# wangyunpeng139/3_ORB_SLAM3_SelfNote

Measured on AMD Instinct MI355X. Metric: frames/sec ORB extract+match, 752x480, higher is better.
Workload: dtype u8; 1 GPU; BASELINE configs[2]: extract + SearchByProjection match, 1000x1000 candidates, synthetic frame stream; image=752x480, nfeatures=1000, nlevels=8, batch=256, distinct_frames_per_gpu=2048, streams=4

## Files before the change

3_orb_slam3_selfnote_amd/csrc/orb_common.h:

```cpp
#pragma once
#include <stdint.h>
#include <stddef.h>

#define ORB_EDGE_THRESHOLD 19
#define ORB_PATCH_SIZE 31
#define ORB_HALF_PATCH 15
#define ORB_MIN_BORDER 16
#define ORB_DISC_PIXELS 749
#define ORB_MAXL 16

#define FAST_TILE_PITCH 80
#define FAST_TILE_COLS 65
#define FAST_TILE_ROWS 76
#define FAST_S_PITCH 64

#define FAST_REC_WORDS 32
#define FAST_REC_GROUP_WORDS 8
#define FAST_REC_CELL_WORDS 4

#define RESIZE_ROWS_MAX 16
#define RESIZE_REC_GROUP_WORDS 4
#define RESIZE_REC_WORDS (RESIZE_REC_GROUP_WORDS + 4 * RESIZE_ROWS_MAX)

#define BLUR_TILE_INTERIOR 0x100u
#define BLUR_TILE_WHOLE_STORES 0x200u

#ifndef ORB_DESCRIBE_K
#define ORB_DESCRIBE_K 8
#endif
#define ORB_DESCRIBE_GROUPS(totalKp, K) ((((totalKp) + (K) - 1) / (K) + 3) / 4 > 1 ? (((totalKp) + (K) - 1) / (K) + 3) / 4 : 1)

__host__ __device__ constexpr int clamp_count(int n, int cap) { return (n > 0 ? n : 0) < cap ? (n > 0 ? n : 0) : cap; }
static_assert(clamp_count(-1, 8) == 0 && clamp_count(0, 8) == 0 && clamp_count(5, 8) == 5 && clamp_count(8, 8) == 8 && clamp_count(9, 8) == 8, "clamp_count");
static_assert(clamp_count(-1, 0) == 0 && clamp_count(0, 0) == 0 && clamp_count(1, 0) == 0, "clamp_count: cap == 0");

struct LiveCount {
  const int32_t *dev; int stride; int konst;
  __device__ __forceinline__ int at(int p, int cap) const { return dev ? clamp_count(dev[(size_t)p * stride], cap) : konst; }
};

struct LevelGeom {
  int w, h;
  int pitch;
  int bpitch;
  size_t off;
  size_t boff;
  int maxBorderX, maxBorderY;
  int nCols, nRows, wCell, hCell;
  int cellCap;
  int cellBase;
  int slotBase;
  int N;
  int nIni;
  float hX;
  int candBase;
  int candCap;
  int kpBase, kpCap;
  float scale;
  float kpsize;
  int xtabBase, ytabBase;
  int resizeRows;
  int resizeSrcRows;
  int resizeTPitch;
  int resizeRecBase;
  int tilesX, tilesY, tileBase;
  uint32_t rowTileMagic;
};

#define CHAIN_TILE 32
#define CHAIN_NT 1024
struct ChainTile {
  uint16_t level, pad;
  uint16_t x[ORB_MAXL], y[ORB_MAXL], w[ORB_MAXL], h[ORB_MAXL];
};

struct FrameParams {
  LevelGeom geom[ORB_MAXL];
  int nlevels;
  int nframes;
  int iniTh, minTh;
  int lap0, lap1;
  const uint8_t *img0;
  size_t img0_stride, img0_frame_stride;
  uint8_t *pyr;    size_t pyr_fs;
  uint8_t *blur;   size_t blur_fs;
  uint32_t *cellCnt; int cell_fs;
  uint32_t *slots;   size_t slot_fs;
  uint32_t *cand;    int cand_fs;
  uint16_t *knode;
  uint32_t *lkp;     int lkp_fs;
  uint16_t *lrank;
  int32_t *lcnt;
  int32_t *candCnt;
  const int2 *xtab, *ytab;
  const int8_t *disc;
  const uint32_t *tiles;
  uint32_t magicCells, magicTiles, magicKpBlk;
  int totalTiles;
  int totalCells;
  int totalGroups;
  uint32_t magicGroups;
  const uint32_t *fastRecs;
  const uint32_t *resizeRecs;
  int totalKp;
  int octCap;
  const ChainTile *chain;
  int chainBuf0, chainBuf1;
  void *out_kps;
  uint8_t *out_desc;
  int32_t *out_counts;
  int cap;
};
```

3_orb_slam3_selfnote_amd/csrc/orb_kernels.h:

```cpp
#pragma once
#include <hip/hip_runtime.h>
#include <type_traits>
#include "orb_common.h"
#include "orb_fast_score.h"
#include "orb_sincos.h"

#define WAVE 64

__constant__ __attribute__((aligned(16))) int8_t c_pattern[1024] = {
#include "../../include/orb_pattern_data.inc"
};

struct DiscTab { uint32_t w[64][6]; };
constexpr int kDiscUmax[16] = {15, 15, 15, 15, 14, 14, 14, 13, 13, 12, 11, 10, 9, 8, 6, 3};
constexpr DiscTab make_disc_tab() {
  DiscTab t{};
  int n = 0;
  for (int v = -15; v <= 15; v++) {
    const int d = kDiscUmax[v < 0 ? -v : v];
    for (int u = -d; u <= d; u++) {
      const int lane = n & 63, k = n >> 6;
      t.w[lane][k >> 2] |= (uint32_t)(uint8_t)(int8_t)u << (8 * (k & 3));
      t.w[lane][3 + (k >> 2)] |= (uint32_t)(uint8_t)(int8_t)v << (8 * (k & 3));
      n++;
// ... 530 lines not shown
        const unsigned long long bK = __builtin_amdgcn_ballot_w64(keep);
        const uint32_t rank = (uint32_t)nkept + (uint32_t)lane_rank(bK);
        if (keep && rank < cellCap) slots[rank] = ((uint32_t)(S - 1) << 24) | yxv;
        nkept += __popcll(bK);
      };
      for (int y0 = 0; y0 < ch; y0 += 2 * rpi, off += 2 * stepB, yr += 2 * rpi, yx += (uint32_t)rpi << 13) {
        const int SA = sS[off], SB = sS[off + stepB];
        const bool candA = ((tt - SA) & yr) < 0, candB = ((tt - SB) & (yr + rpi)) < 0;
        const unsigned long long bA = __builtin_amdgcn_ballot_w64(candA), bB = __builtin_amdgcn_ballot_w64(candB);
        if (bA != 0ull) walk(candA, SA, off, y0 + sub, yx);
        if (bB != 0ull) walk(candB, SB, off + stepB, y0 + rpi + sub, yx + ((uint32_t)rpi << 12));
      }
    }
    FSTAMP(2);
    if (nkept > 0 || detection == 1 || P.minTh >= P.iniTh) break;
    t = P.minTh;
    wave_lds_order();
  }
  if (lane == 0) *cellCnt = (uint32_t)min(nkept, (int)cellCap);
  FSTAMP(7);
}

#ifdef OCT_STAMPS
#define OSTAMP(i) do { const long long t_ = __builtin_readcyclecounter(); if (threadIdx.x == 0 && g_fast_stamps) g_fast_stamps[(size_t)blockIdx.x * 8 + (i)] += (unsigned int)(t_ - ot0); ot0 = t_; } while (0)
#else
#define OSTAMP(i) do {} while (0)
#endif
struct OctNode { short ulx, urx, uly, bry; };

#ifndef OCT_REGKEYS
#define OCT_REGKEYS 4096
#endif
template <int NT, bool CELLS_LDS>
__global__ __launch_bounds__(NT) void k_octree(FrameParams P, uint32_t *cellOffScratch) {
  extern __shared__ __align__(16) uint8_t smem[];
#ifdef OCT_STAMPS
  long long ot0 = __builtin_readcyclecounter();
#endif
  const int CAP = P.octCap;
  unsigned long long *best = reinterpret_cast<unsigned long long *>(smem);
  uint32_t *chcnt = reinterpret_cast<uint32_t *>(smem);
  int32_t *chpos = reinterpret_cast<int32_t *>(smem + 16 * (size_t)CAP);
  OctNode *nodeA = reinterpret_cast<OctNode *>(smem + 32 * (size_t)CAP);
  OctNode *nodeB = nodeA + CAP;
  uint32_t *cntA = reinterpret_cast<uint32_t *>(nodeB + CAP);
  uint32_t *cntB = cntA + CAP;
  int32_t *npos = reinterpret_cast<int32_t *>(cntB + CAP);
  int32_t *rankOf = npos + CAP;
  uint32_t *incl = reinterpret_cast<uint32_t *>(rankOf + CAP);
  uint32_t *sflag = incl + CAP;
  uint32_t *sw = sflag + CAP;
  __shared__ int shI[8];

  const int tid = threadIdx.x, lane = tid & 63, wid = tid >> 6;
  constexpr int NW = NT / 64;
  const int level = (int)(blockIdx.x / (unsigned)P.nframes), frame = (int)(blockIdx.x - (unsigned)level * (unsigned)P.nframes);
  const LevelGeom G = P.geom[level];
  int32_t *lcnt = P.lcnt + ((size_t)frame * P.nlevels + level) * 2;
  uint32_t *cand = P.cand + (size_t)frame * P.cand_fs + G.candBase;
  uint16_t *knode = P.knode + (size_t)frame * P.cand_fs + G.candBase;
  constexpr int PER = OCT_REGKEYS / NT, REGN = PER * NT;
  uint32_t rc[PER > 0 ? PER : 1], rk[PER > 0 ? PER : 1];
#pragma unroll
  for (int j = 0; j < PER; j++) { rc[j] = 0u; rk[j] = 0u; }
  auto for_keys = [&](int n_, auto f) {
#pragma unroll
    for (int j = 0; j < PER; j++) {
      if (j * NT >= n_) break;
      const int k = tid + j * NT;
      if (k < n_) f(k, rc[j], rk[j]);
    }
    for (int k = REGN + tid; k < n_; k += NT) {
      uint32_t c = cand[k], nd = knode[k];
      f(k, c, nd);
      knode[k] = (uint16_t)nd;
    }
  };

  const int ncell = G.nCols * G.nRows;
  const uint32_t *cellCnt = P.cellCnt + (size_t)frame * P.cell_fs + G.cellBase;
  uint32_t *cellOffG = cellOffScratch + (size_t)frame * P.cell_fs + G.cellBase;
  uint32_t *cellOffL = sw + (NT / 64 + 2);
  uint32_t carry = 0;
  for (int base = 0; base < ncell; base += NT) {
    int i = base + tid;
// ... 25 lines not shown
          const int mid = (lo + hi + 1) >> 1;
          if (cellOffL[mid] <= (uint32_t)k) lo = mid; else hi = mid - 1;
        }
        return slots[(size_t)lo * G.cellCap + ((uint32_t)k - cellOffL[lo])];
      };
#pragma unroll
      for (int j = 0; j < PER; j++) {
        if (j * NT >= n) break;
        const int k = tid + j * NT;
        if (k < n) { rc[j] = fetch(k); cand[k] = rc[j]; }
      }
      for (int k = REGN + tid; k < n; k += NT) cand[k] = fetch(k);
      __syncthreads();
    } else {
      for (int cidx = wid; cidx < ncell; cidx += NW) {
        uint32_t cnt = cellCnt[cidx], off = cellOffG[cidx];
        for (uint32_t j = lane; j < cnt; j += 64)
          if (off + j < (uint32_t)n) cand[off + j] = slots[(size_t)cidx * G.cellCap + j];
      }
      __syncthreads();
#pragma unroll
      for (int j = 0; j < PER; j++) {
        if (j * NT >= n) break;
        const int k = tid + j * NT;
        if (k < n) rc[j] = cand[k];
      }
    }
  }
  OSTAMP(0);

  const int nIni = G.nIni;
  const float hX = G.hX;
  const int Hrect = G.maxBorderY - ORB_MIN_BORDER;
  for (int i = tid; i < nIni; i += NT) chcnt[i] = 0;
  __syncthreads();
  for_keys(n, [&](int, uint32_t &c, uint32_t &nd) {
    int r = (int)((float)(c & 0xfff) / hX);
    r = min(max(r, 0), nIni - 1);
    nd = (uint32_t)r;
    atomicAdd(&chcnt[r], 1u);
  });
  __syncthreads();
  if (tid == 0) {
    int L = 0;
    for (int r = 0; r < nIni; r++) {
      uint32_t cn = chcnt[r];
      if (cn > 0) {
        OctNode nd;
        nd.ulx = (short)(int)(hX * (float)r);
        nd.urx = (short)(int)(hX * (float)(r + 1));
        nd.uly = 0;
        nd.bry = (short)Hrect;
        nodeA[L] = nd;
        cntA[L] = cn;
        chpos[r] = L;
        L++;
      }
    }
    shI[0] = L;
  }
  __syncthreads();
  for_keys(n, [&](int, uint32_t &, uint32_t &nd) { nd = (uint32_t)chpos[nd]; });
  int L = shI[0];
  __syncthreads();
  OSTAMP(1);

  const int N = G.N;
  bool careful = false;
  OctNode *nodes = nodeA, *nodesN = nodeB;
  uint32_t *cnts = cntA, *cntsN = cntB;
  for (int guard = 0; guard < 64; guard++) {
    const int prevSize = L;
    for (int i = tid; i < 4 * L; i += NT) chcnt[i] = 0;
    if (tid == 0) { shI[1] = 0; shI[2] = 0x7fffffff; }
    __syncthreads();
    for_keys(n, [&](int, uint32_t &c, uint32_t &nd) {
      if (cnts[nd] > 1) {
        OctNode o = nodes[nd];
        int x = c & 0xfff, y = (c >> 12) & 0xfff;
        int hx = (o.urx - o.ulx + 1) >> 1, hy = (o.bry - o.uly + 1) >> 1;
        int q = (x < o.ulx + hx ? 0 : 1) + (y < o.uly + hy ? 0 : 2);
        atomicAdd(&chcnt[nd * 4 + q], 1u);
      }
    });
    __syncthreads();
    OSTAMP(2);
    int mstar, Eproc, Lnew;
    const bool fusedScan = !careful && L < 1024;
    if (fusedScan) {
      for (int i = tid; i < L; i += NT) {
        const bool e = cnts[i] > 1;
        const uint32_t c = e ? (chcnt[i * 4] > 0) + (chcnt[i * 4 + 1] > 0) + (chcnt[i * 4 + 2] > 0) + (chcnt[i * 4 + 3] > 0) : 0u;
        sflag[i] = (e ? 1u : 0u) | (c << 10) | ((e ? 0u : 1u) << 22);
      }
      __syncthreads();
      const uint32_t tot = lds_excl_scan<NT>(sflag, L, sw);
      mstar = (int)(tot & 1023u) - 1;
      Eproc = (int)((tot >> 10) & 4095u);
      Lnew = Eproc + (int)(tot >> 22);
    } else {
    if (!careful) {
      for (int i = tid; i < L; i += NT) sflag[i] = cnts[i] > 1 ? 1u : 0u;
      __syncthreads();
      uint32_t nX = lds_excl_scan<NT>(sflag, L, sw);
      for (int i = tid; i < L; i += NT) rankOf[i] = cnts[i] > 1 ? (int)sflag[i] : -1;
      if (tid == 0) shI[3] = (int)nX;
    } else {
      uint32_t myX = 0;
      for (int i0 = 0; i0 < L; i0 += NT / 4) {
        const int i = i0 + (tid >> 2), part = tid & 3;
        const uint32_t ci = i < L ? cnts[i] : 0u;
        int r = 0;
        if (ci > 1)
          for (int j = part; j < L; j += 4) {
            const uint32_t cj = cnts[j];
            r += (cj > 1 && (cj > ci || (cj == ci && j < i))) ? 1 : 0;
          }
        r += __builtin_amdgcn_update_dpp(0, r, 0xb1, 0xf, 0xf, true);
        r += __builtin_amdgcn_update_dpp(0, r, 0x4e, 0xf, 0xf, true);
        if (i < L && part == 0) {
          rankOf[i] = ci > 1 ? r : -1;
          if (ci > 1) myX++;
        }
      }
      myX = (uint32_t)wave_sum_i32((int)myX);
      if (lane == 0 && myX) atomicAdd(&shI[1], (int)myX);
      __syncthreads();
      if (tid == 0) { shI[3] = shI[1]; shI[1] = 0; }
    }
    __syncthreads();
    const int nX = shI[3];
    for (int i = tid; i < L; i += NT) {
      int r = rankOf[i];
      if (r >= 0) {
        uint32_t c = (chcnt[i * 4] > 0) + (chcnt[i * 4 + 1] > 0) + (chcnt[i * 4 + 2] > 0) + (chcnt[i * 4 + 3] > 0);
        incl[r] = c;
      }
    }
    __syncthreads();
    lds_excl_scan<NT>(incl, nX, sw);
    if (careful) {
      for (int i = tid; i < L; i += NT) {
        int r = rankOf[i];
        if (r >= 0) {
          uint32_t c = (chcnt[i * 4] > 0) + (chcnt[i * 4 + 1] > 0) + (chcnt[i * 4 + 2] > 0) + (chcnt[i * 4 + 3] > 0);
          int after = L + (int)(incl[r] + c) - (r + 1);
          if (after >= N) atomicMin(&shI[2], r);
        }
      }
    }
    __syncthreads();
    mstar = nX - 1;
    if (careful && shI[2] != 0x7fffffff) mstar = shI[2];
    for (int i = tid; i < L; i += NT) {
      int r = rankOf[i];
      bool proc = r >= 0 && r <= mstar;
      sflag[i] = proc ? 0u : 1u;
      if (r == mstar && r >= 0) {
        uint32_t c = (chcnt[i * 4] > 0) + (chcnt[i * 4 + 1] > 0) + (chcnt[i * 4 + 2] > 0) + (chcnt[i * 4 + 3] > 0);
        shI[4] = (int)(incl[r] + c);
      }
    }
    if (tid == 0 && nX == 0) shI[4] = 0;
    __syncthreads();
    Eproc = shI[4];
    uint32_t nUnproc = lds_excl_scan<NT>(sflag, L, sw);
    Lnew = Eproc + (int)nUnproc;
    }
    OSTAMP(3);
    for (int i = tid; i < L; i += NT) {
      OctNode o = nodes[i];
      bool proc;
      uint32_t childrenBefore, unprocBefore;
      if (fusedScan) {
        const uint32_t pk = sflag[i];
        proc = cnts[i] > 1; childrenBefore = (pk >> 10) & 4095u; unprocBefore = pk >> 22;
      } else {
        const int r = rankOf[i];
        proc = r >= 0 && r <= mstar; childrenBefore = proc ? incl[r] : 0u; unprocBefore = sflag[i];
      }
      if (proc) {
        uint32_t c0 = chcnt[i * 4], c1 = chcnt[i * 4 + 1], c2 = chcnt[i * 4 + 2], c3 = chcnt[i * 4 + 3];
        uint32_t c = (c0 > 0) + (c1 > 0) + (c2 > 0) + (c3 > 0);
        int pos = Eproc - (int)(childrenBefore + c);
        int hx = (o.urx - o.ulx + 1) >> 1, hy = (o.bry - o.uly + 1) >> 1;
        int nexp = 0;
        uint32_t cc[4] = {c0, c1, c2, c3};
#pragma unroll
        for (int q = 3; q >= 0; q--) {
          if (cc[q] > 0) {
            OctNode ch;
            ch.ulx = (short)((q & 1) ? o.ulx + hx : o.ulx);
            ch.urx = (short)((q & 1) ? o.urx : o.ulx + hx);
            ch.uly = (short)((q & 2) ? o.uly + hy : o.uly);
            ch.bry = (short)((q & 2) ? o.bry : o.uly + hy);
            if (pos < CAP) { nodesN[pos] = ch; cntsN[pos] = cc[q]; }
            chpos[i * 4 + q] = pos;
            nexp += cc[q] > 1 ? 1 : 0;
            pos++;
          } else {
            chpos[i * 4 + q] = -1;
          }
        }
        if (nexp) atomicAdd(&shI[1], nexp);
        npos[i] = -1;
      } else {
        int pos = Eproc + (int)unprocBefore;
        if (pos < CAP) { nodesN[pos] = o; cntsN[pos] = cnts[i]; }
        npos[i] = pos;
      }
    }
    __syncthreads();
    OSTAMP(4);
    for_keys(n, [&](int, uint32_t &c, uint32_t &nd) {
      int np = npos[nd];
      if (np < 0) {
        OctNode o = nodes[nd];
        int x = c & 0xfff, y = (c >> 12) & 0xfff;
        int hx = (o.urx - o.ulx + 1) >> 1, hy = (o.bry - o.uly + 1) >> 1;
        int q = (x < o.ulx + hx ? 0 : 1) + (y < o.uly + hy ? 0 : 2);
        np = chpos[nd * 4 + q];
      }
      nd = (uint32_t)(uint16_t)np;
    });
    const int nToExpand = shI[1];
    __syncthreads();
    OSTAMP(5);
    { OctNode *t = nodes; nodes = nodesN; nodesN = t; }
    { uint32_t *t = cnts; cnts = cntsN; cntsN = t; }
    L = min(Lnew, CAP);
    if (Lnew >= N || Lnew == prevSize) break;
    if (!careful && Lnew + nToExpand * 3 > N) careful = true;
  }

  for (int i = tid; i < L; i += NT) best[i] = 0ull;
  __syncthreads();
  for_keys(n, [&](int k, uint32_t &c, uint32_t &nd) {
    const unsigned long long key = ((unsigned long long)(c >> 24) << 32) | (unsigned long long)(0xffffffffu - (uint32_t)k);
    atomicMax(&best[nd], key);
  });
  __syncthreads();
  uint32_t *lkp = P.lkp + (size_t)frame * P.lkp_fs + G.kpBase;
  uint16_t *lrank = P.lrank + (size_t)frame * P.lkp_fs + G.kpBase;
  const int Lout = min(L, G.kpCap);
  for_keys(n, [&](int k, uint32_t &c, uint32_t &nd) {
    const unsigned long long key = ((unsigned long long)(c >> 24) << 32) | (unsigned long long)(0xffffffffu - (uint32_t)k);
    if ((int)nd < Lout && best[nd] == key) {
      lkp[nd] = c;
      float xs = (float)((int)(c & 0xfff) + ORB_MIN_BORDER);
      if (level != 0) xs = xs * G.scale;
      const bool lap = xs >= (float)P.lap0 && xs <= (float)P.lap1;
      sflag[nd] = lap ? 1u : 0u;
    }
  });
  __syncthreads();
  for (int i = tid; i < Lout; i += NT) incl[i] = sflag[i];
  __syncthreads();
  uint32_t nLap = lds_excl_scan<NT>(sflag, Lout, sw);
  for (int i = tid; i < Lout; i += NT) {
    uint32_t f = incl[i];
    uint32_t rank = f ? sflag[i] : (uint32_t)i - sflag[i];
    lrank[i] = (uint16_t)((f << 15) | (rank & 0x7fff));
  }
  if (tid == 0) { lcnt[0] = Lout; lcnt[1] = (int)nLap; }
  OSTAMP(6);
}

// ... 908 lines not shown
```

3_orb_slam3_selfnote_amd/csrc/orbhip.hip:

```cpp
#include <hip/hip_runtime.h>
#include <math.h>
#include <cmath>
#include <assert.h>
#include <stdio.h>
#include <stdlib.h>
#include <string.h>
#include <string>
#include <vector>
#include <algorithm>
#include <type_traits>
#include <mutex>
#include <map>
#include <chrono>

#include "../../include/orbhip.h"
#include "orb_kernels.h"
#include "orb_match_kernels.h"
#include "orb_match_mfma.h"
#include "orb_project_kernels.h"
#include "orb_stereo_kernels.h"
#include "orb_depth_kernels.h"
#include "orb_rig_stereo_kernels.h"
#include "orb_newpoints_kernels.h"
#include "orb_fuse_kernels.h"
// ... 25 lines not shown
  hipError_t reserve(size_t need) {
    if (need <= bytes) return hipSuccess;
    const double t0 = trace_alloc() ? wall_ms() : 0.0;
    if (p) (void)hipFree(p);
    const double t1 = trace_alloc() ? wall_ms() : 0.0;
    p = nullptr;
    const size_t old = bytes;
    bytes = 0;
    hipError_t e = hipMalloc(&p, need);
    if (e == hipSuccess) bytes = need;
    if (trace_alloc()) fprintf(stderr, "orbhip-alloc: device buffer %zu -> %zu bytes: hipFree %.3f ms, hipMalloc %.3f ms\n", old, need, t1 - t0, wall_ms() - t1);
    return e;
  }
  void release() {
    if (p) (void)hipFree(p);
    p = nullptr;
    bytes = 0;
  }
};

}

struct orbx_handle {
  int device = 0;
  int nfeatures = 0, nlevels = 0, iniThFAST = 0, minThFAST = 0;
  double scaleFactor = 0;
  std::vector<float> mvScaleFactor, mvInvScaleFactor, mvLevelSigma2, mvInvLevelSigma2;
  std::vector<int> mnFeaturesPerLevel;
  int umax[ORB_HALF_PATCH + 1];
  int rows = 0, cols = 0, max_batch = 0;
  std::vector<LevelGeom> geom;
  size_t pyr_fs = 0, blur_fs = 0, slot_fs = 0;
  bool octCellsLds = false;
  int chainTiles = 0, chainBuf0 = 0, chainBuf1 = 0;
  size_t chainLds = 0;
  size_t octLds = 0;
  int cell_fs = 0, cand_fs = 0, lkp_fs = 0, totalTiles = 0, totalCells = 0, totalGroups = 0, totalKp = 0, octCap = 0;
  int maxKeypoints = 0;
  DevBuf d_pyr, d_blur, d_cellCnt, d_cellOff, d_slots, d_cand, d_knode, d_lkp, d_lrank, d_lcnt, d_candCnt, d_fastRecs, d_resizeRecs, d_tiles, d_xtab,
      d_ytab, d_disc, d_chain;
  DevBuf d_img, d_okps;
  hipStream_t stream = nullptr;
  float host_us[4] = {0, 0, 0, 0};
  FrameParams last{};
  bool have_last = false;
  hipEvent_t last_done = nullptr;
  bool last_pending = false;
  bool in_capture = false;
  DevBuf stereo[7];
  DevBuf stereo_batch[3];
  DevBuf maps[2];
  int maps_rows = 0, maps_cols = 0;
  void *pin_in = nullptr, *pin_out = nullptr;
  size_t pin_in_bytes = 0, pin_out_bytes = 0;
  DevBuf d_pyrpack; void *pin_pyr = nullptr; size_t pin_pyr_bytes = 0;
  hipGraphExec_t graph = nullptr;
  struct { int rows = 0, cols = 0, lap0 = 0, lap1 = 0, icap = 0; const void *pin_in = nullptr, *pin_out = nullptr, *d_img = nullptr, *d_okps = nullptr, *d_pyr = nullptr; } graph_key;
  bool graph_ok = true;
  bool profiling = false;
  hipEvent_t ev[PROF_DEPTH][6] = {};
  int prof_head = 0;
  bool ev_ok = false;
  float stage_ms[5] = {0, 0, 0, 0, 0};
  bool stage_valid = false;
  std::string err;
};

static hipError_t copy_on(hipStream_t s, void *dst, const void *src, size_t bytes, hipMemcpyKind kind) {
  hipError_t e = hipMemcpyAsync(dst, src, bytes, kind, s);
  return e != hipSuccess ? e : hipStreamSynchronize(s);
}
static hipError_t join_last(orbx_handle *h) {
  if (h->last_pending) { hipError_t e = hipStreamWaitEvent(h->stream, h->last_done, 0); if (e != hipSuccess) return e; }
// ... 126 lines not shown
      h->umax[v] = v0;
      ++v0;
    }
  }
  std::vector<int8_t> disc;
  for (int v = -ORB_HALF_PATCH; v <= ORB_HALF_PATCH; v++) {
    const int d = h->umax[v < 0 ? -v : v];
    for (int u = -d; u <= d; u++) { disc.push_back((int8_t)u); disc.push_back((int8_t)v); }
  }
  if ((int)disc.size() != 2 * ORB_DISC_PIXELS) { delete h; return nullptr; }
  {
    const DiscTab ref = make_disc_tab();
    for (int i = 0; i < ORB_DISC_PIXELS; i++) {
      const int lane = i & 63, k = i >> 6;
      const int8_t u = (int8_t)(ref.w[lane][k >> 2] >> (8 * (k & 3))), v = (int8_t)(ref.w[lane][3 + (k >> 2)] >> (8 * (k & 3)));
      if (u != disc[2 * i] || v != disc[2 * i + 1]) { delete h; return nullptr; }
    }
  }
  if (hipStreamCreateWithFlags(&h->stream, hipStreamNonBlocking) != hipSuccess) { delete h; return nullptr; }
  if (h->d_disc.reserve(disc.size()) != hipSuccess ||
      copy_on(h->stream, h->d_disc.p, disc.data(), disc.size(), hipMemcpyHostToDevice) != hipSuccess) {
    (void)hipStreamDestroy(h->stream);
    delete h;
    return nullptr;
  }
  return h;
}

void orbx_destroy(orbx_t *h) {
  if (!h) return;
  (void)hipSetDevice(h->device);
  if (h->stream) (void)hipStreamSynchronize(h->stream);
  DevBuf *bufs[] = {&h->d_pyr, &h->d_blur, &h->d_cellCnt, &h->d_cellOff, &h->d_slots, &h->d_cand, &h->d_knode, &h->d_lkp,
                    &h->d_lrank, &h->d_lcnt, &h->d_candCnt, &h->d_fastRecs, &h->d_resizeRecs, &h->d_tiles, &h->d_xtab, &h->d_ytab, &h->d_disc, &h->d_chain, &h->d_img, &h->d_okps};
  for (DevBuf *b : bufs) b->release();
  for (DevBuf &b : h->stereo) b.release();
  for (DevBuf &b : h->stereo_batch) b.release();
  for (DevBuf &b : h->maps) b.release();
  if (h->graph) (void)hipGraphExecDestroy(h->graph);
  if (h->last_done) (void)hipEventDestroy(h->last_done);
  if (h->pin_in) (void)hipHostFree(h->pin_in);
  if (h->pin_pyr) (void)hipHostFree(h->pin_pyr);
  h->d_pyrpack.release();
  if (h->pin_out) (void)hipHostFree(h->pin_out);
  if (h->ev_ok)
    for (auto &set : h->ev)
      for (auto &e : set) (void)hipEventDestroy(e);
  if (h->stream) (void)hipStreamDestroy(h->stream);
  delete h;
}

const char *orbx_last_error(const orbx_t *h) { return h ? h->err.c_str() : "null handle"; }
int orbx_get_levels(const orbx_t *h) { return h ? h->nlevels : ORBX_E_ARG; }
float orbx_get_scale_factor(const orbx_t *h) { return h ? (float)h->scaleFactor : 0.f; }

int orbx_get_scale_tables(const orbx_t *h, float *sf, float *isf, float *s2, float *is2) {
  if (!h) return ORBX_E_ARG;
  for (int i = 0; i < h->nlevels; i++) {
    if (sf) sf[i] = h->mvScaleFactor[i];
    if (isf) isf[i] = h->mvInvScaleFactor[i];
    if (s2) s2[i] = h->mvLevelSigma2[i];
    if (is2) is2[i] = h->mvInvLevelSigma2[i];
  }
  return h->nlevels;
}

int orbx_get_features_per_level(const orbx_t *h, int *n) {
// ... 284 lines not shown
            const size_t area = (size_t)T.w[l] * T.h[l];
            if (l < L) { if (l & 1) b1 = std::max(b1, area); else b0 = std::max(b0, area); }
            if (l == 0) break;
            tab += (size_t)T.w[l] + T.h[l];
            const int sw = g[l - 1].w, sh = g[l - 1].h;
            const int2 *xt = &xtab[g[l].xtabBase], *yt = &ytab[g[l].ytabBase];
            int nx0 = sw, nx1 = 0, ny0 = sh, ny1 = 0;
            for (int x = x0; x <= x1; x++) { nx0 = std::min(nx0, xt[x].x); nx1 = std::max(nx1, std::min(xt[x].x + 1, sw - 1)); }
            for (int y = y0; y <= y1; y++) {
              ny0 = std::min(ny0, std::min(std::max(yt[y].x, 0), sh - 1));
              ny1 = std::max(ny1, std::min(std::max(yt[y].x + 1, 0), sh - 1));
            }
            x0 = nx0; x1 = nx1; y0 = ny0; y1 = ny1;
          }
          tabMax = std::max(tabMax, tab);
          tilesC.push_back(T);
        }
    b0 = align_up(b0, 16); b1 = align_up(b1, 16);
    const size_t lds = b0 + b1 + sizeof(int2) * tabMax;
    h->chainTiles = 0;
    if (!tilesC.empty() && lds <= 64 * 1024 && b1 <= 16384 && b0 <= 65536 && tilesC.size() < 65536) {
      bool ok = true;
      for (const ChainTile &T : tilesC)
        for (int l = 1; l <= T.level; l++) ok = ok && (size_t)T.w[l] * T.h[l] < 16384;
      if (ok) {
        XCHECK(h, h->d_chain.reserve(sizeof(ChainTile) * tilesC.size()));
        XCHECK(h, copy_on(h->stream, h->d_chain.p, tilesC.data(), sizeof(ChainTile) * tilesC.size(), hipMemcpyHostToDevice));
        h->chainTiles = (int)tilesC.size(); h->chainBuf0 = (int)b0; h->chainBuf1 = (int)b1; h->chainLds = lds;
      }
    }
  }
  int maxCells = 1;
  for (int l = 0; l < nl; l++) maxCells = std::max(maxCells, g[l].nCols * g[l].nRows);
  size_t lds = 72 * (size_t)octCap + 128;
  if (lds > 160 * 1024 - 256) { h->err = "nfeatures too large for the LDS-resident octree"; return ORBX_E_ARG; }
  h->octCellsLds = lds + 4 * ((size_t)maxCells + 1) <= 96 * 1024;
  if (h->octCellsLds) lds += 4 * ((size_t)maxCells + 1);
  h->octLds = lds;
  if (lds > ORB_LDS_LIMIT) { h->err = "octree LDS state exceeds 160 KiB"; return ORBX_E_ARG; }
  h->rows = rows;
  h->cols = cols;
  h->max_batch = max_batch;
  h->have_last = false;
  return h->maxKeypoints;
}

void orbx_set_profiling(orbx_t *h, int enable) {
  if (!h) return;
  h->profiling = enable != 0;
  h->prof_head = 0;
  h->stage_valid = false;
  if (h->profiling && !h->ev_ok) {
    (void)hipSetDevice(h->device);
    bool ok = true;
    for (auto &set : h->ev)
      for (auto &e : set) ok = ok && hipEventCreate(&e) == hipSuccess;
    h->ev_ok = ok;
  }
}

int orbx_get_stage_ms(orbx_t *h, float *ms, int cap) {
  if (!h || !ms || !h->profiling || !h->ev_ok || !h->stage_valid || h->prof_head <= 0) return 0;
  const int nb = std::min(h->prof_head, PROF_DEPTH), n = std::min(cap, 5);
  if (hipEventSynchronize(h->ev[(h->prof_head - 1) % PROF_DEPTH][5]) != hipSuccess) return 0;
  for (int i = 0; i < n; i++) ms[i] = 0.f;
  for (int b = 0; b < nb; b++) {
    const int slot = (h->prof_head - 1 - b) % PROF_DEPTH;
// ... 26 lines not shown
  P.minTh = h->minThFAST;
  P.lap0 = lap0;
  P.lap1 = lap1;
  P.img0 = d_images;
  P.img0_stride = stride;
  P.img0_frame_stride = frame_stride;
  P.pyr = (uint8_t *)h->d_pyr.p;       P.pyr_fs = h->pyr_fs;
  P.blur = (uint8_t *)h->d_blur.p;     P.blur_fs = h->blur_fs;
  P.cellCnt = (uint32_t *)h->d_cellCnt.p; P.cell_fs = h->cell_fs;
  P.slots = (uint32_t *)h->d_slots.p;  P.slot_fs = h->slot_fs;
  P.cand = (uint32_t *)h->d_cand.p;    P.cand_fs = h->cand_fs;
  P.knode = (uint16_t *)h->d_knode.p;
  P.lkp = (uint32_t *)h->d_lkp.p;      P.lkp_fs = h->lkp_fs;
  P.lrank = (uint16_t *)h->d_lrank.p;
  P.lcnt = (int32_t *)h->d_lcnt.p;
  P.candCnt = (int32_t *)h->d_candCnt.p;
  P.xtab = (const int2 *)h->d_xtab.p;
  P.ytab = (const int2 *)h->d_ytab.p;
  P.disc = (const int8_t *)h->d_disc.p;
  P.totalTiles = h->totalTiles;
  P.totalCells = h->totalCells;
  P.fastRecs = (const uint32_t *)h->d_fastRecs.p;
  P.resizeRecs = (const uint32_t *)h->d_resizeRecs.p;
  P.totalGroups = h->totalGroups;
  P.magicGroups = magic_div((uint32_t)std::max(h->totalGroups, 1));
  P.tiles = (const uint32_t *)h->d_tiles.p;
  P.magicCells = magic_div((uint32_t)std::max(h->totalCells, 1));
  P.magicTiles = magic_div((uint32_t)std::max(h->totalTiles, 1));
  const bool wide = (long long)h->nlevels * nframes <= 32;
  const int describeGroups = wide ? ORB_DESCRIBE_GROUPS(h->totalKp, 1) : ORB_DESCRIBE_GROUPS(h->totalKp, ORB_DESCRIBE_K);
  P.magicKpBlk = magic_div((uint32_t)describeGroups);
  P.totalKp = h->totalKp;
  P.octCap = h->octCap;
  P.chain = (const ChainTile *)h->d_chain.p; P.chainBuf0 = h->chainBuf0; P.chainBuf1 = h->chainBuf1;
  P.out_kps = d_kps;
  P.out_desc = d_desc;
  P.out_counts = d_counts;
  P.cap = cap;
  const bool prof = h->profiling && h->ev_ok;
  hipEvent_t *pev = h->ev[h->prof_head % PROF_DEPTH];
  if (prof) XCHECK(h, hipEventRecord(pev[0], s));
  const bool printForms = getenv("ORBHIP_PRINT_EXTRACT_FORMS") != nullptr;
  std::string pyrForm = h->nlevels == 1 ? "none" : "";
  if (wide && h->chainTiles > 0) { hipLaunchKernelGGL(k_pyramid_chain, dim3(h->chainTiles * nframes), dim3(CHAIN_NT), h->chainLds, s, P); pyrForm = "chain"; }
  else
  for (int l = 1; l < h->nlevels; l++) {
    const LevelGeom &G = h->geom[l], &Gs = h->geom[l - 1];
    const int rowBytes = (int)align_up((size_t)Gs.w + 4, 16);
    size_t lds;
    (void)resize_form(G, Gs, &lds);
    const int tPitch = G.resizeTPitch;
    const bool twoPass = tPitch > 0;
    hipLaunchKernelGGL(k_resize, dim3(((G.h + G.resizeRows - 1) / G.resizeRows) * nframes), dim3(256), lds, s, P, l, rowBytes, tPitch, G.resizeSrcRows);
    if (printForms) pyrForm += std::string(l > 1 ? "," : "") + (!twoPass ? "1p" : G.resizeRows == 16 ? "2p16" : "2p8");
  }
  if (prof) XCHECK(h, hipEventRecord(pev[1], s));
  if (h->totalGroups > 0) hipLaunchKernelGGL(k_fast, dim3(h->totalGroups * nframes), dim3(FAST_NT), 0, s, P);
  if (prof) XCHECK(h, hipEventRecord(pev[2], s));
  if (wide) {
    if (h->octCellsLds) hipLaunchKernelGGL((k_octree<1024, true>), dim3(h->nlevels * nframes), dim3(1024), h->octLds, s, P, (uint32_t *)h->d_cellOff.p);
    else hipLaunchKernelGGL((k_octree<1024, false>), dim3(h->nlevels * nframes), dim3(1024), h->octLds, s, P, (uint32_t *)h->d_cellOff.p);
  } else {
    if (h->octCellsLds) hipLaunchKernelGGL((k_octree<256, true>), dim3(h->nlevels * nframes), dim3(256), h->octLds, s, P, (uint32_t *)h->d_cellOff.p);
    else hipLaunchKernelGGL((k_octree<256, false>), dim3(h->nlevels * nframes), dim3(256), h->octLds, s, P, (uint32_t *)h->d_cellOff.p);
  }
  if (prof) XCHECK(h, hipEventRecord(pev[3], s));
  hipLaunchKernelGGL(k_blur, dim3(h->totalTiles * nframes), dim3(256), 0, s, P);
  if (prof) XCHECK(h, hipEventRecord(pev[4], s));
  if (wide) hipLaunchKernelGGL(k_describe<1>, dim3(describeGroups * nframes), dim3(256), 0, s, P);
  else hipLaunchKernelGGL(k_describe<ORB_DESCRIBE_K>, dim3(describeGroups * nframes), dim3(256), 0, s, P);
  if (prof) { XCHECK(h, hipEventRecord(pev[5], s)); h->prof_head++; h->stage_valid = true; }
  XCHECK(h, hipGetLastError());
  if (printForms) {
    int aligned0 = 0;
    for (int f = 0; f < nframes; f++) aligned0 += (((uintptr_t)(d_images + (size_t)f * frame_stride) | (uintptr_t)stride) & 3u) == 0;
    const LevelGeom &G0 = h->geom[0];
    const int blur0dma = G0.w >= 160 && G0.h >= 40 && (G0.w & 15) == 0 ? aligned0 : 0;
    fprintf(stderr, "orbhip: extract nframes %d pyramid %s octree %d/%s aligned0 %d blur0dma %d describe %d\n", nframes, pyrForm.c_str(), wide ? 1024 : 256,
            h->octCellsLds ? "lds" : "global", aligned0, blur0dma, wide ? 1 : ORB_DESCRIBE_K);
  }
  h->last = P;
  h->have_last = true;
  if (!h->in_capture) {
    if (!h->last_done) XCHECK(h, hipEventCreateWithFlags(&h->last_done, hipEventDisableTiming));
    XCHECK(h, hipEventRecord(h->last_done, s));
    h->last_pending = true;
  }
  return 0;
}

int orbx_extract(orbx_t *h, const uint8_t *image, int rows, int cols, size_t stride, int lap0, int lap1,
                 orbx_keypoint_t *keypoints, uint8_t *descriptors, int cap, int *n_out) {
  if (!h) return ORBX_E_ARG;
  if (n_out) *n_out = 0;
  if (!image || rows <= 0 || cols <= 0) return ORBX_E_EMPTY;
  if (stride < (size_t)cols || !n_out) return ORBX_E_ARG;
  int rc = orbx_configure(h, rows, cols, h->rows == rows && h->cols == cols ? h->max_batch : 1);
  if (rc < 0) return rc;
  const int icap = h->maxKeypoints;
  const size_t dstride = align_up((size_t)cols, 64);
  XCHECK(h, hipSetDevice(h->device));
  XCHECK(h, h->d_img.reserve(dstride * rows));
  const size_t in_bytes = dstride * rows, kp_bytes = sizeof(orbx_keypoint_t) * (size_t)icap, de_bytes = 32 * (size_t)icap;
  const size_t kp_off = 64, de_off = kp_off + align_up(kp_bytes, 64), out_bytes = de_off + de_bytes;
  XCHECK(h, h->d_okps.reserve(out_bytes));
  if (h->pin_in_bytes < in_bytes) {
    if (h->pin_in) (void)hipHostFree(h->pin_in);
    h->pin_in = nullptr; h->pin_in_bytes = 0;
    XCHECK(h, hipHostMalloc(&h->pin_in, in_bytes, hipHostMallocDefault));
    h->pin_in_bytes = in_bytes;
  }
  if (h->pin_out_bytes < out_bytes) {
// ... 5041 lines not shown
```

Baseline: 317,300 frames/s.

## Precompute octree quadtree counts via lookup tables instead of per-round key passes

Adds host-built per-level lookup tables that map each keypoint x/y to its initial node and a 5-level quadtree path. The octree kernel bins keypoints once into an LDS count pyramid and derives child counts from it during splitting, so nodes carry compact codes instead of rescanning and relabelling every key each round. Keys are labelled only at the end, or when splitting goes past the table depth. It also sets waves_per_eu(4) on the octree kernel and reserves extra LDS for the table, which may lower occupancy or fall back to the old path.

```diff
diff --git a/3_orb_slam3_selfnote_amd/csrc/orb_common.h b/3_orb_slam3_selfnote_amd/csrc/orb_common.h
--- a/3_orb_slam3_selfnote_amd/csrc/orb_common.h
+++ b/3_orb_slam3_selfnote_amd/csrc/orb_common.h
@@ -39,6 +39,10 @@
   __device__ __forceinline__ int at(int p, int cap) const { return dev ? clamp_count(dev[(size_t)p * stride], cap) : konst; }
 };
 
+#define OCT_D 5
+#define OCT_PYR_OFF(nIni, d) ((uint32_t)(nIni) * (((1u << (2 * OCT_D + 2)) - (4u << (2 * (d)))) / 3u))
+#define OCT_TABLE_BYTES(nIni) ((size_t)((2u * OCT_PYR_OFF(nIni, 0) + 2u * (uint32_t)(nIni) + 3u) & ~3u))
+
 struct LevelGeom {
   int w, h;
   int pitch;
@@ -56,6 +60,7 @@
   int candBase;
   int candCap;
   int kpBase, kpCap;
+  int octTabX, octTabY;
   float scale;
   float kpsize;
   int xtabBase, ytabBase;
@@ -104,6 +109,8 @@
   const uint32_t *resizeRecs;
   int totalKp;
   int octCap;
+  int octHead;
+  const uint8_t *octTab;
   const ChainTile *chain;
   int chainBuf0, chainBuf1;
   void *out_kps;
diff --git a/3_orb_slam3_selfnote_amd/csrc/orb_kernels.h b/3_orb_slam3_selfnote_amd/csrc/orb_kernels.h
--- a/3_orb_slam3_selfnote_amd/csrc/orb_kernels.h
+++ b/3_orb_slam3_selfnote_amd/csrc/orb_kernels.h
@@ -586,7 +586,8 @@
 #define OCT_REGKEYS 4096
 #endif
 template <int NT, bool CELLS_LDS>
-__global__ __launch_bounds__(NT) void k_octree(FrameParams P, uint32_t *cellOffScratch) {
+__global__ __launch_bounds__(NT) __attribute__((amdgpu_waves_per_eu(4))) void k_octree(
+FrameParams P, uint32_t *cellOffScratch) {
   extern __shared__ __align__(16) uint8_t smem[];
 #ifdef OCT_STAMPS
   long long ot0 = __builtin_readcyclecounter();
@@ -595,7 +596,7 @@
   unsigned long long *best = reinterpret_cast<unsigned long long *>(smem);
   uint32_t *chcnt = reinterpret_cast<uint32_t *>(smem);
   int32_t *chpos = reinterpret_cast<int32_t *>(smem + 16 * (size_t)CAP);
-  OctNode *nodeA = reinterpret_cast<OctNode *>(smem + 32 * (size_t)CAP);
+  OctNode *nodeA = reinterpret_cast<OctNode *>(smem + (size_t)P.octHead);
   OctNode *nodeB = nodeA + CAP;
   uint32_t *cntA = reinterpret_cast<uint32_t *>(nodeB + CAP);
   uint32_t *cntB = cntA + CAP;
@@ -605,6 +606,9 @@
   uint32_t *sflag = incl + CAP;
   uint32_t *sw = sflag + CAP;
   __shared__ int shI[8];
+  uint16_t *pyr = reinterpret_cast<uint16_t *>(smem);
+  uint16_t *codeA = reinterpret_cast<uint16_t *>(npos), *codeB = codeA + CAP;
+  bool codes = P.octTab != nullptr;
 
   const int tid = threadIdx.x, lane = tid & 63, wid = tid >> 6;
   constexpr int NW = NT / 64;
@@ -696,6 +700,33 @@
   const int nIni = G.nIni;
   const float hX = G.hX;
   const int Hrect = G.maxBorderY - ORB_MIN_BORDER;
+  if (n > 65535) codes = false;
+  if (codes) {
+    uint32_t *bins = reinterpret_cast<uint32_t *>(smem);
+    for (int i = tid; i < (nIni << (2 * OCT_D - 1)); i += NT) bins[i] = 0u;
+    if (tid == 0) shI[5] = 0;
+    __syncthreads();
+    const uint8_t *tabX = P.octTab + G.octTabX, *tabY = P.octTab + G.octTabY;
+    const int Wrect = G.maxBorderX - ORB_MIN_BORDER;
+    for_keys(n, [&](int, uint32_t &c, uint32_t &nd) {
+      const int x = min((int)(c & 0xfff), Wrect), y = min((int)((c >> 12) & 0xfff), Hrect);
+      nd = ((uint32_t)tabX[x] << OCT_D) | (uint32_t)tabY[y];
+      atomicAdd(&bins[nd >> 1], 1u << ((nd & 1u) << 4));
+    });
+    __syncthreads();
+#pragma unroll
+    for (int d = OCT_D - 1; d >= 0; d--) {
+      const uint16_t *fine = pyr + OCT_PYR_OFF(nIni, d + 1);
+      uint16_t *coarse = pyr + OCT_PYR_OFF(nIni, d);
+      for (int e = tid; e < (nIni << (2 * d)); e += NT) {
+        const int ix = e >> d, iy = e & ((1 << d) - 1);
+        const uint32_t w0 = *reinterpret_cast<const uint32_t *>(fine + ((2 * ix) << (d + 1)) + 2 * iy);
+        const uint32_t w1 = *reinterpret_cast<const uint32_t *>(fine + ((2 * ix + 1) << (d + 1)) + 2 * iy);
+        coarse[e] = (uint16_t)((w0 & 0xffffu) + (w0 >> 16) + (w1 & 0xffffu) + (w1 >> 16));
+      }
+      __syncthreads();
+    }
+  } else {
   for (int i = tid; i < nIni; i += NT) chcnt[i] = 0;
   __syncthreads();
   for_keys(n, [&](int, uint32_t &c, uint32_t &nd) {
@@ -705,10 +736,11 @@
     atomicAdd(&chcnt[r], 1u);
   });
   __syncthreads();
+  }
   if (tid == 0) {
     int L = 0;
     for (int r = 0; r < nIni; r++) {
-      uint32_t cn = chcnt[r];
+      uint32_t cn = codes ? (uint32_t)pyr[OCT_PYR_OFF(nIni, 0) + r] : chcnt[r];
       if (cn > 0) {
         OctNode nd;
         nd.ulx = (short)(int)(hX * (float)r);
@@ -717,14 +749,14 @@
         nd.bry = (short)Hrect;
         nodeA[L] = nd;
         cntA[L] = cn;
-        chpos[r] = L;
+        if (codes) codeA[L] = (uint16_t)(r << 5); else chpos[r] = L;
         L++;
       }
     }
     shI[0] = L;
   }
   __syncthreads();
-  for_keys(n, [&](int, uint32_t &, uint32_t &nd) { nd = (uint32_t)chpos[nd]; });
+  if (!codes) for_keys(n, [&](int, uint32_t &, uint32_t &nd) { nd = (uint32_t)chpos[nd]; });
   int L = shI[0];
   __syncthreads();
   OSTAMP(1);
@@ -733,12 +765,48 @@
   bool careful = false;
   OctNode *nodes = nodeA, *nodesN = nodeB;
   uint32_t *cnts = cntA, *cntsN = cntB;
+  uint16_t *ncode = codeA, *ncodeN = codeB;
+  auto label_keys = [&]() {
+    for (int w = tid; w < 4 * L; w += NT) {
+      const int i = w >> 2, part = w & 3;
+      const uint32_t code = ncode[i];
+      const int up = OCT_D - (int)(code >> 13), side = 1 << up;
+      const int x0 = (int)((code >> 5) & 255u) << up, y0 = (int)(code & 31u) << up;
+      if (up == 0) { if (part == 0) pyr[(x0 << OCT_D) + y0] = (uint16_t)i; }
+      else
+        for (int cx = part; cx < side; cx += 4) {
+          uint32_t *col = reinterpret_cast<uint32_t *>(pyr + ((x0 + cx) << OCT_D) + y0);
+          for (int j = 0; j < side / 2; j++) col[j] = (uint32_t)i * 0x10001u;
+        }
+    }
+    __syncthreads();
+    for_keys(n, [&](int, uint32_t &, uint32_t &nd) { nd = (uint32_t)pyr[nd]; });
+    __syncthreads();
+  };
+  auto child_counts = [&](int i, uint32_t &c0, uint32_t &c1, uint32_t &c2, uint32_t &c3) {
+    if (codes) {
+      const uint32_t code = ncode[i];
+      const int d = min((int)(code >> 13), OCT_D - 1), ix = (int)((code >> 5) & 255u), iy = (int)(code & 31u);
+      const uint16_t *fine = pyr + OCT_PYR_OFF(nIni, d + 1);
+      const uint32_t w0 = *reinterpret_cast<const uint32_t *>(fine + ((2 * ix) << (d + 1)) + 2 * iy);
+      const uint32_t w1 = *reinterpret_cast<const uint32_t *>(fine + ((2 * ix + 1) << (d + 1)) + 2 * iy);
+      c0 = w0 & 0xffffu; c1 = w1 & 0xffffu; c2 = w0 >> 16; c3 = w1 >> 16;
+    } else {
+      c0 = chcnt[i * 4]; c1 = chcnt[i * 4 + 1]; c2 = chcnt[i * 4 + 2]; c3 = chcnt[i * 4 + 3];
+    }
+  };
+  auto child_nodes = [&](int i) -> uint32_t {
+    uint32_t c0, c1, c2, c3;
+    child_counts(i, c0, c1, c2, c3);
+    return (c0 > 0) + (c1 > 0) + (c2 > 0) + (c3 > 0);
+  };
   for (int guard = 0; guard < 64; guard++) {
     const int prevSize = L;
-    for (int i = tid; i < 4 * L; i += NT) chcnt[i] = 0;
+    if (codes && shI[5] != 0) { label_keys(); codes = false; }
+    if (!codes) for (int i = tid; i < 4 * L; i += NT) chcnt[i] = 0;
     if (tid == 0) { shI[1] = 0; shI[2] = 0x7fffffff; }
     __syncthreads();
-    for_keys(n, [&](int, uint32_t &c, uint32_t &nd) {
+    if (!codes) for_keys(n, [&](int, uint32_t &c, uint32_t &nd) {
       if (cnts[nd] > 1) {
         OctNode o = nodes[nd];
         int x = c & 0xfff, y = (c >> 12) & 0xfff;
@@ -754,7 +822,7 @@
     if (fusedScan) {
       for (int i = tid; i < L; i += NT) {
         const bool e = cnts[i] > 1;
-        const uint32_t c = e ? (chcnt[i * 4] > 0) + (chcnt[i * 4 + 1] > 0) + (chcnt[i * 4 + 2] > 0) + (chcnt[i * 4 + 3] > 0) : 0u;
+        const uint32_t c = e ? child_nodes(i) : 0u;
         sflag[i] = (e ? 1u : 0u) | (c << 10) | ((e ? 0u : 1u) << 22);
       }
       __syncthreads();
@@ -797,7 +865,7 @@
     for (int i = tid; i < L; i += NT) {
       int r = rankOf[i];
       if (r >= 0) {
-        uint32_t c = (chcnt[i * 4] > 0) + (chcnt[i * 4 + 1] > 0) + (chcnt[i * 4 + 2] > 0) + (chcnt[i * 4 + 3] > 0);
+        uint32_t c = child_nodes(i);
         incl[r] = c;
       }
     }
@@ -807,7 +875,7 @@
       for (int i = tid; i < L; i += NT) {
         int r = rankOf[i];
         if (r >= 0) {
-          uint32_t c = (chcnt[i * 4] > 0) + (chcnt[i * 4 + 1] > 0) + (chcnt[i * 4 + 2] > 0) + (chcnt[i * 4 + 3] > 0);
+          uint32_t c = child_nodes(i);
           int after = L + (int)(incl[r] + c) - (r + 1);
           if (after >= N) atomicMin(&shI[2], r);
         }
@@ -821,7 +889,7 @@
       bool proc = r >= 0 && r <= mstar;
       sflag[i] = proc ? 0u : 1u;
       if (r == mstar && r >= 0) {
-        uint32_t c = (chcnt[i * 4] > 0) + (chcnt[i * 4 + 1] > 0) + (chcnt[i * 4 + 2] > 0) + (chcnt[i * 4 + 3] > 0);
+        uint32_t c = child_nodes(i);
         shI[4] = (int)(incl[r] + c);
       }
     }
@@ -844,8 +912,11 @@
         proc = r >= 0 && r <= mstar; childrenBefore = proc ? incl[r] : 0u; unprocBefore = sflag[i];
       }
       if (proc) {
-        uint32_t c0 = chcnt[i * 4], c1 = chcnt[i * 4 + 1], c2 = chcnt[i * 4 + 2], c3 = chcnt[i * 4 + 3];
+        uint32_t c0, c1, c2, c3;
+        child_counts(i, c0, c1, c2, c3);
         uint32_t c = (c0 > 0) + (c1 > 0) + (c2 > 0) + (c3 > 0);
+        const uint32_t code = codes ? (uint32_t)ncode[i] : 0u;
+        const uint32_t dN = (code >> 13) + 1u, ixN = 2u * ((code >> 5) & 255u), iyN = 2u * (code & 31u);
         int pos = Eproc - (int)(childrenBefore + c);
         int hx = (o.urx - o.ulx + 1) >> 1, hy = (o.bry - o.uly + 1) >> 1;
         int nexp = 0;
@@ -859,24 +930,27 @@
             ch.uly = (short)((q & 2) ? o.uly + hy : o.uly);
             ch.bry = (short)((q & 2) ? o.bry : o.uly + hy);
             if (pos < CAP) { nodesN[pos] = ch; cntsN[pos] = cc[q]; }
-            chpos[i * 4 + q] = pos;
+            if (codes) { if (pos < CAP) ncodeN[pos] = (uint16_t)((dN << 13) | ((ixN + (q & 1)) << 5) | (iyN + (q >> 1))); }
+            else chpos[i * 4 + q] = pos;
             nexp += cc[q] > 1 ? 1 : 0;
             pos++;
           } else {
-            chpos[i * 4 + q] = -1;
+            if (!codes) chpos[i * 4 + q] = -1;
           }
         }
         if (nexp) atomicAdd(&shI[1], nexp);
-        npos[i] = -1;
+        if (codes) { if (nexp && dN == OCT_D) shI[5] = 1; }
+        else npos[i] = -1;
       } else {
         int pos = Eproc + (int)unprocBefore;
         if (pos < CAP) { nodesN[pos] = o; cntsN[pos] = cnts[i]; }
-        npos[i] = pos;
+        if (codes) { if (pos < CAP) ncodeN[pos] = ncode[i]; }
+        else npos[i] = pos;
       }
     }
     __syncthreads();
     OSTAMP(4);
-    for_keys(n, [&](int, uint32_t &c, uint32_t &nd) {
+    if (!codes) for_keys(n, [&](int, uint32_t &c, uint32_t &nd) {
       int np = npos[nd];
       if (np < 0) {
         OctNode o = nodes[nd];
@@ -892,11 +966,13 @@
     OSTAMP(5);
     { OctNode *t = nodes; nodes = nodesN; nodesN = t; }
     { uint32_t *t = cnts; cnts = cntsN; cntsN = t; }
+    { uint16_t *t = ncode; ncode = ncodeN; ncodeN = t; }
     L = min(Lnew, CAP);
     if (Lnew >= N || Lnew == prevSize) break;
     if (!careful && Lnew + nToExpand * 3 > N) careful = true;
   }
 
+  if (codes) label_keys();
   for (int i = tid; i < L; i += NT) best[i] = 0ull;
   __syncthreads();
   for_keys(n, [&](int k, uint32_t &c, uint32_t &nd) {
diff --git a/3_orb_slam3_selfnote_amd/csrc/orbhip.hip b/3_orb_slam3_selfnote_amd/csrc/orbhip.hip
--- a/3_orb_slam3_selfnote_amd/csrc/orbhip.hip
+++ b/3_orb_slam3_selfnote_amd/csrc/orbhip.hip
@@ -81,13 +81,15 @@
   std::vector<LevelGeom> geom;
   size_t pyr_fs = 0, blur_fs = 0, slot_fs = 0;
   bool octCellsLds = false;
+  bool octCodes = false;
+  size_t octHead = 0;
   int chainTiles = 0, chainBuf0 = 0, chainBuf1 = 0;
   size_t chainLds = 0;
   size_t octLds = 0;
   int cell_fs = 0, cand_fs = 0, lkp_fs = 0, totalTiles = 0, totalCells = 0, totalGroups = 0, totalKp = 0, octCap = 0;
   int maxKeypoints = 0;
   DevBuf d_pyr, d_blur, d_cellCnt, d_cellOff, d_slots, d_cand, d_knode, d_lkp, d_lrank, d_lcnt, d_candCnt, d_fastRecs, d_resizeRecs, d_tiles, d_xtab,
-      d_ytab, d_disc, d_chain;
+      d_ytab, d_disc, d_chain, d_octTab;
   DevBuf d_img, d_okps;
   hipStream_t stream = nullptr;
   float host_us[4] = {0, 0, 0, 0};
@@ -280,7 +282,7 @@
   (void)hipSetDevice(h->device);
   if (h->stream) (void)hipStreamSynchronize(h->stream);
   DevBuf *bufs[] = {&h->d_pyr, &h->d_blur, &h->d_cellCnt, &h->d_cellOff, &h->d_slots, &h->d_cand, &h->d_knode, &h->d_lkp,
-                    &h->d_lrank, &h->d_lcnt, &h->d_candCnt, &h->d_fastRecs, &h->d_resizeRecs, &h->d_tiles, &h->d_xtab, &h->d_ytab, &h->d_disc, &h->d_chain, &h->d_img, &h->d_okps};
+                    &h->d_lrank, &h->d_lcnt, &h->d_candCnt, &h->d_fastRecs, &h->d_resizeRecs, &h->d_tiles, &h->d_xtab, &h->d_ytab, &h->d_disc, &h->d_chain, &h->d_octTab, &h->d_img, &h->d_okps};
   for (DevBuf *b : bufs) b->release();
   for (DevBuf &b : h->stereo) b.release();
   for (DevBuf &b : h->stereo_batch) b.release();
@@ -631,7 +633,48 @@
   }
   int maxCells = 1;
   for (int l = 0; l < nl; l++) maxCells = std::max(maxCells, g[l].nCols * g[l].nRows);
-  size_t lds = 72 * (size_t)octCap + 128;
+  {
+    int maxIni = 0;
+    for (int l = 0; l < nl; l++) maxIni = std::max(maxIni, g[l].nIni);
+    size_t limit = ORB_LDS_LIMIT;
+    if (const char *e = getenv("ORBHIP_OCTREE_TABLE_LIMIT")) limit = (size_t)strtoul(e, nullptr, 10);
+    const size_t tabBytes = align_up(OCT_TABLE_BYTES(std::max(maxIni, 1)), 16);
+    h->octCodes = maxIni >= 1 && (maxIni << OCT_D) <= 256 && octCap <= 65535 && tabBytes <= limit;
+    h->octHead = 32 * (size_t)octCap;
+    if (h->octCodes && tabBytes > h->octHead) {
+      if (tabBytes + 40 * (size_t)octCap + 128 + 4 * ((size_t)maxCells + 1) <= 32 * 1024) h->octHead = tabBytes;
+      else h->octCodes = false;
+    }
+    if (h->octCodes) {
+      std::vector<uint8_t> tab;
+      auto walk = [](int v, int ul, int ur) {
+        int bits = 0;
+        for (int d = 0; d < OCT_D; d++) {
+          const int half = (ur - ul + 1) >> 1;
+          const int b = v < ul + half ? 0 : 1;
+          if (b) ul = ul + half; else ur = ul + half;
+          bits = (bits << 1) | b;
+        }
+        return bits;
+      };
+      for (int l = 0; l < nl; l++) {
+        LevelGeom &G = g[l];
+        G.octTabX = G.octTabY = (int)tab.size();
+        if (G.nIni < 1) continue;
+        const int Wrect = G.maxBorderX - ORB_MIN_BORDER, Hrect = G.maxBorderY - ORB_MIN_BORDER;
+        for (int x = 0; x <= Wrect; x++) {
+          const int r = std::min(std::max((int)((float)x / G.hX), 0), G.nIni - 1);
+          tab.push_back((uint8_t)((r << OCT_D) | walk(x, (int)(G.hX * (float)r), (int)(G.hX * (float)(r + 1)))));
+        }
+        G.octTabY = (int)tab.size();
+        for (int y = 0; y <= Hrect; y++) tab.push_back((uint8_t)walk(y, 0, Hrect));
+      }
+      h->geom = g;
+      XCHECK(h, h->d_octTab.reserve(std::max<size_t>(tab.size(), 1)));
+      if (!tab.empty()) XCHECK(h, copy_on(h->stream, h->d_octTab.p, tab.data(), tab.size(), hipMemcpyHostToDevice));
+    }
+  }
+  size_t lds = h->octHead + 40 * (size_t)octCap + 128;
   if (lds > 160 * 1024 - 256) { h->err = "nfeatures too large for the LDS-resident octree"; return ORBX_E_ARG; }
   h->octCellsLds = lds + 4 * ((size_t)maxCells + 1) <= 96 * 1024;
   if (h->octCellsLds) lds += 4 * ((size_t)maxCells + 1);
@@ -724,6 +767,8 @@
   P.magicKpBlk = magic_div((uint32_t)describeGroups);
   P.totalKp = h->totalKp;
   P.octCap = h->octCap;
+  P.octHead = (int)h->octHead;
+  P.octTab = h->octCodes ? (const uint8_t *)h->d_octTab.p : nullptr;
   P.chain = (const ChainTile *)h->d_chain.p; P.chainBuf0 = h->chainBuf0; P.chainBuf1 = h->chainBuf1;
   P.out_kps = d_kps;
   P.out_desc = d_desc;
@@ -768,8 +813,8 @@
     for (int f = 0; f < nframes; f++) aligned0 += (((uintptr_t)(d_images + (size_t)f * frame_stride) | (uintptr_t)stride) & 3u) == 0;
     const LevelGeom &G0 = h->geom[0];
     const int blur0dma = G0.w >= 160 && G0.h >= 40 && (G0.w & 15) == 0 ? aligned0 : 0;
-    fprintf(stderr, "orbhip: extract nframes %d pyramid %s octree %d/%s aligned0 %d blur0dma %d describe %d\n", nframes, pyrForm.c_str(), wide ? 1024 : 256,
-            h->octCellsLds ? "lds" : "global", aligned0, blur0dma, wide ? 1 : ORB_DESCRIBE_K);
+    fprintf(stderr, "orbhip: extract nframes %d pyramid %s octree %d/%s aligned0 %d blur0dma %d describe %d rounds %s octLds %zu octCap %d\n", nframes, pyrForm.c_str(), wide ? 1024 : 256,
+            h->octCellsLds ? "lds" : "global", aligned0, blur0dma, wide ? 1 : ORB_DESCRIBE_K, h->octCodes ? "codes" : "keys", h->octLds, h->octCap);
   }
   h->last = P;
   h->have_last = true;
```

Result: faster. 326,700 frames/s (median of 6 runs) (+2.9%).
